# ostadabbas/TePose

Hardware: AMD Instinct MI355X
Metric: 16-frame windows/sec (whole node) (higher is better)
Workload: dtype f32 via 3 fp16 MFMAs on hi+lo halves (22 bits/operand, fp32 acc); exact-f32 MFMA run = value_exact_fp32; 1 GPU; cfg-C synthetic [8192,16,2133] fp32 windows per GPU, TePose n_layers=2 hidden=1024, random-init weights, synthetic SMPL tables, H36M-14 joint path; seqlen=16, parallelism=clip-sharded dp1

## Files before the change

include/tepose_amd.h:

```cpp
#ifndef TEPOSE_AMD_H
#define TEPOSE_AMD_H

#include <stddef.h>
#include <stdint.h>

#ifdef __cplusplus
extern "C" {
#endif

#define TEPOSE_ABI_VERSION 1

#define TEPOSE_E_ARG (-1)
#define TEPOSE_E_SHAPE (-2)
#define TEPOSE_E_WORKSPACE (-3)
#define TEPOSE_E_STATE (-4)
#define TEPOSE_E_TIMEOUT (-5)

#define TEPOSE_FEAT 2048
#define TEPOSE_THETA 85
#define TEPOSE_INPUT 2133
#define TEPOSE_NVERT 6890
#define TEPOSE_NJOINT 24

typedef struct tepose_model tepose_model;
// ... 62 lines not shown
int tepose_project_frame_pair(const tepose_model* m, const float* feat_prev, const float* feat_new, long feat_ld, const float* theta_prev,
                              long theta_ld, int B, float* out_prev, long out_prev_ld, float* out_new, long out_new_ld, void* workspace,
                              size_t ws_bytes, void* stream);
int tepose_window_step(const tepose_model* m, const float* feat_prev, const float* feat_new, long feat_ld, const float* theta_prev, long theta_ld,
                       float* out_prev, long out_prev_ld, float* newest, long newest_ld, const float* ring_base, int ring, int first_slot,
                       long clip_stride, int B, int T, const void* jreg_packed, float* theta, float* verts, float* kp_3d, float* kp_2d, float* rotmat,
                       void* workspace, size_t ws_bytes, void* pair_workspace, size_t pair_ws_bytes, void* stream);
int tepose_forward_cached(const tepose_model* m, const float* ring_base, int ring, int first_slot,
                          long clip_stride, const float* newest, long newest_ld, int B, int T,
                          const void* jreg_packed, float* theta, float* verts, float* kp_3d,
                          float* kp_2d, float* rotmat, void* workspace, size_t ws_bytes, void* stream);

int tepose_create_vibe(int n_layers, int hidden, tepose_model** out);
int tepose_create_vibe_ex(int n_layers, int hidden, int bidirectional, int add_linear, tepose_model** out);
int tepose_pack_vibe_encoder(tepose_model* m, const float* const* w, int n_w, void* stream);
size_t tepose_vibe_workspace_bytes(const tepose_model* m, int B, int N);
int tepose_vibe_feature_dim(const tepose_model* m);
int tepose_vibe_encoder_fwd(const tepose_model* m, const float* x, int B, int N, int use_residual,
                            float* feat, void* workspace, size_t ws_bytes, void* stream);

int tepose_create_hmr(tepose_model** out);
int tepose_pack_hmr_backbone(tepose_model* m, const float* const* w, int n_w, void* stream);
size_t tepose_hmr_workspace_bytes(const tepose_model* m, int N);
int tepose_hmr_features(const tepose_model* m, const float* x, int N, float* feat, void* workspace, size_t ws_bytes, void* stream);

int tepose_metrics_joints(const float* pred, const float* target, int N, int J, int pelvis_mode,
                          float* mpjpe, float* pa_mpjpe, float* accel, void* stream);
int tepose_smpl_verts_from_theta(const tepose_model* m, const float* theta, int N, float* verts,
                                 void* workspace, size_t ws_bytes, void* stream);
int tepose_smpl_fwd(const tepose_model* m, int pose2rot, const float* pose, const float* betas, int N,
                    float* verts, float* joints49, void* workspace, size_t ws_bytes, void* stream);
int tepose_joints_from_verts(const tepose_model* m, const void* jreg_packed, const float* verts, int N, float* kp_3d, void* stream);
int tepose_smpl_fwd_per_person(const tepose_model* m, const float* pose, const float* betas, int N, float* verts,
                               void* workspace, size_t ws_bytes, void* stream);
int tepose_metrics_verts(const float* pred_verts, const float* target_verts, int N, float* mpvpe,
                         void* stream);

int tepose_filter_one_euro(float* x, int N, int D, float min_cutoff, float beta, float d_cutoff,
                           void* stream);
int tepose_filter_slerp(const float* rotmat_in, float* rotmat_out, int N, int J, double ratio,
                        void* stream);

int tepose_rotmat_to_angle_axis(const float* R, int N, float* aa, void* stream);
int tepose_rot6d_to_rotmat(const float* x6, int N, float* R, void* stream);

size_t tepose_gemm_workspace_bytes(int N, int K);
int tepose_gemm_f32(const float* A, long lda, const float* W, long ldw, const float* bias,
                    float* C, long ldc, int M, int N, int K, int relu_a, void* workspace,
                    size_t ws_bytes, void* stream);

size_t tepose_gemm_h3_workspace_bytes(int M, int N, int K);
int tepose_gemm_h3_f32(const float* A, long lda, const float* W, long ldw, const float* bias, float* C,
                       long ldc, int M, int N, int K, void* workspace, size_t ws_bytes, void* stream);

size_t tepose_conv2d_nhwc_workspace_bytes(int N, int H, int W, int Cin, int Cout, int R);
int tepose_conv2d_nhwc_f32(const float* x, int N, int H, int W, int Cin, const float* w_oihw, const float* bias, int Cout, int R,
                           int stride, int pad, int relu_in, const float* residual, float* y, int exact, void* workspace,
                           size_t ws_bytes, void* stream);
int tepose_maxpool3x3s2_nhwc(const float* x, int N, int H, int W, int C, float* y, void* stream);
int tepose_avgpool7_nhwc(const float* x, int N, int C, float* y, void* stream);
int tepose_hmr_fold_pack(const float* w_oihw, const float* gamma, const float* beta, const float* mean, const float* var, int Cout,
                         int Cin, int R, float* w_out, float* b_out, void* stream);

int tepose_profile_enable(tepose_model* m, int on);
int tepose_profile_read(tepose_model* m, double* total_ms, int* n_launches, double* flops_per_launch);
int tepose_profile_read_gru(tepose_model* m, double* total_ms, int* n_forwards, double* flops_per_forward);
int tepose_profile_read_l1proj(tepose_model* m, double* total_ms, int* n_forwards, double* flops_per_forward);

#ifdef __cplusplus
}
#endif
#endif
```

tepose_amd/_lib.py:

```python
import ctypes
import os
from ctypes import c_uint, POINTER, c_char_p, c_double, c_float, c_int, c_int32, c_long, c_size_t, c_void_p

_HERE = os.path.dirname(os.path.abspath(__file__))
LIB_PATH = (os.environ.get("TEPOSE_AMD_LIB") or os.path.join(_HERE, 'libtepose_hip.so'))

SYMBOLS = [
    'tepose_version', 'tepose_error_string', 'tepose_create', 'tepose_destroy',
    'tepose_packed_bytes', 'tepose_set_blob', 'tepose_adopt_blob', 'tepose_pack_encoder', 'tepose_pack_regressor',
    'tepose_pack_smpl', 'tepose_jreg_packed_bytes', 'tepose_pack_jreg', 'tepose_workspace_bytes',
    'tepose_encoder_fwd', 'tepose_regressor_fwd', 'tepose_forward', 'tepose_gemm_workspace_bytes',
    'tepose_gemm_f32', 'tepose_profile_enable', 'tepose_profile_read', 'tepose_create_vibe', 'tepose_create_vibe_ex', 'tepose_vibe_feature_dim',
    'tepose_pack_vibe_encoder', 'tepose_vibe_workspace_bytes', 'tepose_vibe_encoder_fwd',
    'tepose_metrics_joints', 'tepose_smpl_verts_from_theta', 'tepose_metrics_verts', 'tepose_smpl_fwd', 'tepose_filter_one_euro', 'tepose_filter_slerp', 'tepose_project_frames', 'tepose_project_frame_pair', 'tepose_window_step', 'tepose_forward_cached', 'tepose_profile_read_gru', 'tepose_profile_read_l1proj', 'tepose_gemm_h3_workspace_bytes', 'tepose_gemm_h3_f32',
    'tepose_regressor_fwd_init', 'tepose_rotmat_to_angle_axis', 'tepose_rot6d_to_rotmat',
    'tepose_project_frames_workspace_bytes', 'tepose_smpl_fwd_per_person', 'tepose_joints_from_verts',
    'tepose_status', 'tepose_forward_status', 'tepose_status_peek', 'tepose_fault_code', 'tepose_set_persistent', 'tepose_uses_persistent', 'tepose_build_info',
    'tepose_fp32_ranges', 'tepose_derive_planes', 'tepose_kernel_info', 'tepose_select_kernels', 'tepose_set_option', 'tepose_get_option', 'tepose_debug_set_test_fault', 'tepose_debug_kernel_errors',
    'tepose_create_hmr', 'tepose_pack_hmr_backbone', 'tepose_hmr_workspace_bytes', 'tepose_hmr_features', 'tepose_conv2d_nhwc_workspace_bytes',
    'tepose_conv2d_nhwc_f32', 'tepose_maxpool3x3s2_nhwc', 'tepose_avgpool7_nhwc', 'tepose_hmr_fold_pack',
]

_lib = None


class TeposeError(RuntimeError):
    pass


E_TIMEOUT = -5


class TeposeTimeout(TeposeError):
    """TEPOSE_E_TIMEOUT: a persistent small-batch kernel gave up waiting for its peers (GPU shared or CU-masked);
    the outputs of that forward are NaN.  Engine re-runs on the step-per-launch kernels where it owns the sync point."""


class TeposeKernelFault(TeposeError):
    """(A sibling of TeposeTimeout, not a subclass: the retry loops that catch TeposeTimeout -- run_clips, StreamSession -- must not re-run on it.)
    The fault channel reported code 4: a bounded LDS poll of the barrier-free projection kernel (csrc/gemm_h3s16c.hip) expired.  No wait in that
    kernel depends on another workgroup, so this is a kernel bug or a hardware fault -- not a shared / CU-masked GPU, and the persistent small-batch
    kernels have nothing to do with it.  The forward's outputs are invalid (NaN-poisoned); the handle stays as it is."""


def load():
    global _lib
    if _lib is not None:
        return _lib
    if not os.path.isfile(LIB_PATH):
        raise ImportError(
            'tepose_amd: %s not found. Build it with `python -c "import __graft_entry__ as g; '
            'g.build()"` (hipcc --offload-arch=gfx950). There is no fallback path.' % LIB_PATH)
    lib = ctypes.CDLL(LIB_PATH)
    fp = c_void_p
    lib.tepose_version.restype = c_int
    lib.tepose_error_string.restype = c_char_p
    lib.tepose_error_string.argtypes = [c_int]
    lib.tepose_create.argtypes = [c_int, c_int, POINTER(c_void_p)]
    lib.tepose_destroy.argtypes = [c_void_p]
    lib.tepose_destroy.restype = None
    lib.tepose_packed_bytes.argtypes = [c_void_p]
    lib.tepose_packed_bytes.restype = c_size_t
    lib.tepose_set_blob.argtypes = [c_void_p, fp, c_size_t]
    lib.tepose_adopt_blob.argtypes = [c_void_p]
    lib.tepose_pack_encoder.argtypes = [c_void_p, POINTER(c_void_p), c_int, c_void_p]
    lib.tepose_pack_regressor.argtypes = [c_void_p, POINTER(c_void_p), c_int, c_void_p]
    lib.tepose_pack_smpl.argtypes = [c_void_p, fp, fp, fp, fp, fp, fp, POINTER(c_int32), c_void_p]
    lib.tepose_jreg_packed_bytes.restype = c_size_t
    lib.tepose_pack_jreg.argtypes = [fp, fp, c_void_p]
    lib.tepose_workspace_bytes.argtypes = [c_void_p, c_int, c_int]
    lib.tepose_workspace_bytes.restype = c_size_t
    lib.tepose_encoder_fwd.argtypes = [c_void_p, fp, c_int, c_int, c_int, fp, fp, c_size_t, c_void_p]
    lib.tepose_regressor_fwd.argtypes = [c_void_p, fp, c_int, c_int, fp, fp, fp, fp, fp, fp, fp,
                                         c_size_t, c_void_p]
    lib.tepose_forward.argtypes = [c_void_p, fp, c_int, c_int, fp, fp, fp, fp, fp, fp, fp, c_size_t,
                                   c_void_p]
    lib.tepose_regressor_fwd_init.argtypes = [c_void_p, fp, c_int, c_int, fp, fp, fp, fp, fp, fp, fp, fp, fp, fp,
                                              c_size_t, c_void_p]
    lib.tepose_rotmat_to_angle_axis.argtypes = [fp, c_int, fp, c_void_p]
    lib.tepose_rot6d_to_rotmat.argtypes = [fp, c_int, fp, c_void_p]
    lib.tepose_gemm_workspace_bytes.argtypes = [c_int, c_int]
    lib.tepose_gemm_workspace_bytes.restype = c_size_t
    lib.tepose_gemm_f32.argtypes = [fp, c_long, fp, c_long, fp, fp, c_long, c_int, c_int, c_int, c_int,
                                    fp, c_size_t, c_void_p]
    lib.tepose_create_vibe.argtypes = [c_int, c_int, POINTER(c_void_p)]
    lib.tepose_create_vibe_ex.argtypes = [c_int, c_int, c_int, c_int, POINTER(c_void_p)]
    lib.tepose_vibe_feature_dim.argtypes = [c_void_p]
    lib.tepose_pack_vibe_encoder.argtypes = [c_void_p, POINTER(c_void_p), c_int, c_void_p]
    lib.tepose_vibe_workspace_bytes.argtypes = [c_void_p, c_int, c_int]
    lib.tepose_vibe_workspace_bytes.restype = c_size_t
    lib.tepose_vibe_encoder_fwd.argtypes = [c_void_p, fp, c_int, c_int, c_int, fp, fp, c_size_t, c_void_p]
    lib.tepose_metrics_joints.argtypes = [fp, fp, c_int, c_int, c_int, fp, fp, fp, c_void_p]
    lib.tepose_smpl_verts_from_theta.argtypes = [c_void_p, fp, c_int, fp, fp, c_size_t, c_void_p]
    lib.tepose_metrics_verts.argtypes = [fp, fp, c_int, fp, c_void_p]
    lib.tepose_smpl_fwd.argtypes = [c_void_p, c_int, fp, fp, c_int, fp, fp, fp, c_size_t, c_void_p]
    lib.tepose_smpl_fwd_per_person.argtypes = [c_void_p, fp, fp, c_int, fp, fp, c_size_t, c_void_p]
    lib.tepose_filter_one_euro.argtypes = [fp, c_int, c_int, c_float, c_float, c_float, c_void_p]
    lib.tepose_filter_slerp.argtypes = [fp, fp, c_int, c_int, c_double, c_void_p]
    lib.tepose_project_frames_workspace_bytes.argtypes = [c_void_p, c_int]
    lib.tepose_project_frames_workspace_bytes.restype = c_size_t
    lib.tepose_project_frames.argtypes = [c_void_p, fp, c_long, fp, c_long, c_int, fp, c_long, fp, c_size_t, c_void_p]
    lib.tepose_project_frame_pair.argtypes = [c_void_p, fp, fp, c_long, fp, c_long, c_int, fp, c_long, fp, c_long, fp, c_size_t, c_void_p]
    lib.tepose_window_step.argtypes = [c_void_p, fp, fp, c_long, fp, c_long, fp, c_long, fp, c_long, fp, c_int, c_int, c_long, c_int, c_int, fp, fp, fp, fp, fp, fp,
                                       fp, c_size_t, fp, c_size_t, c_void_p]
    lib.tepose_forward_cached.argtypes = [c_void_p, fp, c_int, c_int, c_long, fp, c_long, c_int, c_int, fp, fp, fp, fp,
                                          fp, fp, fp, c_size_t, c_void_p]
    lib.tepose_gemm_h3_workspace_bytes.argtypes = [c_int, c_int, c_int]
    lib.tepose_gemm_h3_workspace_bytes.restype = c_size_t
    lib.tepose_gemm_h3_f32.argtypes = [fp, c_long, fp, c_long, fp, fp, c_long, c_int, c_int, c_int, fp, c_size_t, c_void_p]
    lib.tepose_fp32_ranges.argtypes = [c_void_p, POINTER(c_size_t), POINTER(c_size_t), c_int]
    lib.tepose_derive_planes.argtypes = [c_void_p, c_void_p]
    lib.tepose_status.argtypes = [c_void_p, c_void_p]
    lib.tepose_forward_status.argtypes = [c_void_p, c_void_p, c_void_p]
    lib.tepose_debug_set_test_fault.argtypes = [c_void_p, c_uint]
    lib.tepose_debug_kernel_errors.restype = c_uint
    lib.tepose_status_peek.argtypes = [c_void_p]
    lib.tepose_fault_code.argtypes = [c_void_p]
    lib.tepose_set_persistent.argtypes = [c_void_p, c_int]
    lib.tepose_uses_persistent.argtypes = [c_void_p, c_int, c_int]
    lib.tepose_joints_from_verts.argtypes = [c_void_p, fp, fp, c_int, fp, c_void_p]
    lib.tepose_profile_enable.argtypes = [c_void_p, c_int]
    lib.tepose_profile_read.argtypes = [c_void_p, POINTER(c_double), POINTER(c_int), POINTER(c_double)]
    lib.tepose_profile_read_gru.argtypes = [c_void_p, POINTER(c_double), POINTER(c_int), POINTER(c_double)]
    lib.tepose_profile_read_l1proj.argtypes = [c_void_p, POINTER(c_double), POINTER(c_int), POINTER(c_double)]
    lib.tepose_create_hmr.argtypes = [POINTER(c_void_p)]
    lib.tepose_pack_hmr_backbone.argtypes = [c_void_p, POINTER(c_void_p), c_int, c_void_p]
    lib.tepose_hmr_workspace_bytes.argtypes = [c_void_p, c_int]
    lib.tepose_hmr_workspace_bytes.restype = c_size_t
    lib.tepose_hmr_features.argtypes = [c_void_p, fp, c_int, fp, fp, c_size_t, c_void_p]
    lib.tepose_conv2d_nhwc_workspace_bytes.argtypes = [c_int] * 6
    lib.tepose_conv2d_nhwc_workspace_bytes.restype = c_size_t
    lib.tepose_conv2d_nhwc_f32.argtypes = [fp, c_int, c_int, c_int, c_int, fp, fp, c_int, c_int, c_int, c_int, c_int, fp, fp, c_int, fp, c_size_t, c_void_p]
    lib.tepose_maxpool3x3s2_nhwc.argtypes = [fp, c_int, c_int, c_int, c_int, fp, c_void_p]
    lib.tepose_avgpool7_nhwc.argtypes = [fp, c_int, c_int, fp, c_void_p]
    lib.tepose_hmr_fold_pack.argtypes = [fp, fp, fp, fp, fp, c_int, c_int, c_int, fp, fp, c_void_p]
    for name in SYMBOLS:
        getattr(lib, name)
    if lib.tepose_version() != 1:
        raise ImportError('tepose_amd: ABI version mismatch (%d)' % lib.tepose_version())
    lib.tepose_build_info.restype = c_char_p
    lib.tepose_kernel_info.restype = c_char_p
    lib.tepose_kernel_info.argtypes = [c_void_p]
    lib.tepose_select_kernels.restype = c_char_p
    lib.tepose_set_option.argtypes = [c_void_p, c_char_p, ctypes.c_long]
    lib.tepose_get_option.argtypes = [c_void_p, c_char_p]
    lib.tepose_get_option.restype = ctypes.c_long
    lib.tepose_select_kernels.argtypes = [c_void_p, c_int, c_int]
    info = (lib.tepose_build_info() or b'').decode()
    if 'packed_fp32=off' not in info:
        import warnings
        warnings.warn('tepose_amd: %s was built WITH packed-fp32 VALU instructions (%r); on a GPU shared by two processes such a '
                      'build returned wrong SMPL vertices in 1-3 %% of the launches (DESIGN.md section 10) -- rebuild with '
                      '__graft_entry__.build()' % (LIB_PATH, info), RuntimeWarning)
    _lib = lib
    return lib


def check(rc, what):
    if rc != 0:
        msg = load().tepose_error_string(rc)
        raise (TeposeTimeout if rc == E_TIMEOUT else TeposeError)('%s failed: %s (code %d)' % (what, msg.decode() if msg else '?', rc))

# ... 5 lines not shown
```

tepose_amd/csrc/api.hip:

```cpp
#include <stdlib.h>
#include <string.h>

#include <new>

#include "plan.h"

using namespace tepose;

static inline void fault_collected(const tepose_model* m) {
  std::lock_guard<std::mutex> g(m->q_mu);
  ++m->collected;
}

static void read_env_knobs(tepose_model* m) {
  m->opt = options_from_env();
  const char* e = getenv("TEPOSE_EXACT_FP32");
  m->split = m->split_env = !(e && atoi(e) != 0);
  e = getenv("TEPOSE_LARGE_BATCH_KERNELS");
  m->large_scaled = !(e && std::string(e) == "twoacc");
  e = getenv("TEPOSE_GRU_STATE");
  m->state_planes = !(e && std::string(e) == "fp32");
  e = getenv("TEPOSE_COLLAPSE_REGRESSOR");
  m->collapse_env = !(e && atoi(e) == 0);
  e = getenv("TEPOSE_S_MIN_B");
// ... 267 lines not shown
}

int tepose_metrics_verts(const float* pred_verts, const float* target_verts, int N, float* mpvpe, void* stream) {
  if (!pred_verts || !target_verts || !mpvpe || N < 1) return TEPOSE_E_ARG;
  CK(launch_metrics_verts(pred_verts, target_verts, N, mpvpe, (hipStream_t)stream));
  return 0;
}

int tepose_filter_one_euro(float* x, int N, int D, float min_cutoff, float beta, float d_cutoff, void* stream) {
  if (!x || N < 1 || D < 1) return TEPOSE_E_ARG;
  CK(launch_one_euro(x, N, D, min_cutoff, beta, d_cutoff, (hipStream_t)stream));
  return 0;
}

int tepose_filter_slerp(const float* rotmat_in, float* rotmat_out, int N, int J, double ratio, void* stream) {
  if (!rotmat_in || !rotmat_out || N < 1 || J < 1) return TEPOSE_E_ARG;
  CK(launch_slerp_smooth(rotmat_in, rotmat_out, N, J, ratio, (hipStream_t)stream));
  return 0;
}

int tepose_rotmat_to_angle_axis(const float* R, int N, float* aa, void* stream) {
  if (!R || !aa || N < 1) return TEPOSE_E_ARG;
  CK(launch_rotmat_to_aa(R, N, aa, (hipStream_t)stream));
  return 0;
}

int tepose_rot6d_to_rotmat(const float* x6, int N, float* R, void* stream) {
  if (!x6 || !R || N < 1) return TEPOSE_E_ARG;
  CK(launch_rot6d_to_rotmat(x6, N, R, (hipStream_t)stream));
  return 0;
}

size_t tepose_gemm_h3_workspace_bytes(int M, int N, int K) {
  if (M < 1 || N < 1 || K < 1) return 0;
  const size_t a = gemm_h3_ws_bytes(M, N, K), b = gemm_h3s_ws_bytes(M, N, K);
  return a > b ? a : b;
}

int tepose_gemm_h3_f32(const float* A, long lda, const float* W, long ldw, const float* bias, float* C, long ldc,
                       int M, int N, int K, void* workspace, size_t ws_bytes, void* stream) {
  if (!A || !W || !C || !workspace || M < 1 || N < 1 || K < 1) return TEPOSE_E_ARG;
  if (K % 32 != 0) return TEPOSE_E_SHAPE;
  if (ws_bytes < gemm_h3_ws_bytes(M, N, K)) return TEPOSE_E_WORKSPACE;
  const char* pe = getenv("TEPOSE_H3S");
  const Options opt = options_from_env();
  if (pe && pe[0] && std::string(pe) != "0" && std::string(pe).rfind("skinny", 0) != 0 && ws_bytes >= gemm_h3s_ws_bytes(M, N, K)) {
    CK(launch_gemm_h3s_f32(A, lda, W, ldw, C, ldc, M, N, K, 256.f, 16384.f, workspace, (hipStream_t)stream, opt, bias, std::string(pe) == "mid" ? 1 : 0));
    return 0;
  }
  CK(launch_gemm_h3_f32(A, lda, W, ldw, bias, C, ldc, M, N, K, workspace, (hipStream_t)stream, opt, pe && std::string(pe) == "skinny" ? 1 : 0));
  return 0;
}

size_t tepose_gemm_workspace_bytes(int N, int K) {
  if (N < 1 || K < 1) return 0;
  return (size_t)round_up(N, 128) * round_up(K, 32) * sizeof(float) + 256;
}

int tepose_gemm_f32(const float* A, long lda, const float* W, long ldw, const float* bias, float* C, long ldc,
                    int M, int N, int K, int relu_a, void* workspace, size_t ws_bytes, void* stream) {
  if (!A || !W || !C || !workspace || M < 1 || N < 1 || K < 1) return TEPOSE_E_ARG;
  if (lda % 4 != 0 || ((uintptr_t)A & 15) != 0 || K % 32 != 0) return TEPOSE_E_SHAPE;
  if (ws_bytes < tepose_gemm_workspace_bytes(N, K)) return TEPOSE_E_WORKSPACE;
  hipStream_t s = (hipStream_t)stream;
  float* wp = (float*)workspace;
  CK((hipError_t)pack(W, ldw, N, K, wp, round_up(N, 128), K, 0, 0, 0, 1, s));
  const GemmArgs g{A, lda, wp, K, C, ldc, bias, nullptr, 0, 1.f, M, N, relu_a};
  CK(launch_gemm(g, s, options_from_env()));
  return 0;
}

}
```

tepose_amd/csrc/common.h:

```cpp
#pragma once
#include <hip/hip_runtime.h>
#include <stdint.h>

namespace tepose {

typedef _Float16 half_t;
constexpr float kLoScale = 2048.f;
__host__ __device__ inline void split_hi_lo(float a, half_t& hi, half_t& lo) {
  hi = (half_t)a;
  lo = (half_t)((a - (float)hi) * kLoScale);
}

constexpr int kFeat = 2048;
constexpr int kTheta = 85;
constexpr int kInput = 2133;
constexpr int kInputP = 2144;
constexpr int kNV = 6890;
constexpr int kNJ = 24;
constexpr int kNPose = 144;
constexpr int kState = 160;
constexpr int kBlendK = 224;
constexpr int kBlendN = 20736;
constexpr int kVertLd = 20672;

// ... 228 lines not shown
  int N, n_iter;
};
hipError_t launch_reg_seq(const RegSeqArgs& a, hipStream_t s);
bool gru_seq_ok(int ndir, int M, int Hp, int T, const Options& o);
int gru_seq_gran_rows(const Options& o);
hipError_t launch_gru_seq(const GruSeqArgs& a, hipStream_t s, const Options& o);
struct GateBatch { GateDir d[3]; };
hipError_t launch_gru_first(const GateBatch& gb, int ndir, int M, int Hp, hipStream_t s, int scaled16 = 0, bool rows16 = false);
hipError_t launch_split_planes(const float* src, long ld, long rows, int K, int Kp, long R, void* hi, void* lo,
                               hipStream_t s, int relu = 0);
struct RowPairSrc { const float* f0; const float* th0; const float* f1; long fld, thld; long B; };
hipError_t launch_split_rows(const float* src, long ld, long rows, int K, int Kp, long R, int fmt16, void* hi, void* lo,
                             float* row_scale, hipStream_t s, bool few, void* zero = nullptr, size_t zero_bytes = 0,
                             int permT = 0, const RowPairSrc* pair = nullptr);
hipError_t launch_gemm_h3_f32(const float* A, long lda, const float* W, long ldw, const float* bias, float* C,
                              long ldc, int M, int N, int K, void* ws, hipStream_t s, const Options& o, int kind = 0);
size_t gemm_h3_ws_bytes(int M, int N, int K);
__host__ __device__ inline long plane16_index(long row, long k, long R) {
  return ((k >> 4) * R + row) * 16 + ((((k >> 3) & 1) ^ ((row >> 3) & 1)) << 3) + (k & 7);
}
constexpr float kStateScale = 16384.f;
struct H3SArgs {
  const half_t *Ah, *Al; long a_kst;
  const half_t *Wh, *Wl; long w_kst;
  int Kp;
  float* C; long ldc;
  const float* bias;
  float inv_scale;
  int M, N;
  const float* row_scale;
  unsigned* status = nullptr;
  unsigned* fault = nullptr;
  unsigned inject = 0;
  int c_blk_hp = 0;
};
struct H3SBatch { H3SArgs p[3]; GateDir gate[3]; int n; int Hp; float state_scale; };
hipError_t launch_gemm_h3s(const H3SArgs& a, hipStream_t s, const Options& o, int tag = 1);
bool gemm_h3s16_ok(const H3SArgs& a);
hipError_t launch_gemm_h3s16c(const H3SArgs& a, hipStream_t s, int tag, int gm);
unsigned h3s16c_read_err();
void h3s16c_warm();
bool gru_step16_ok(const H3SBatch& b);
bool gru_step16_planes_ok(const H3SBatch& b);
hipError_t launch_gru_step16(const H3SBatch& b, hipStream_t s, bool planes, int gm);
unsigned* h3s16c_err_of_device();
bool gemm_h3s_mid_ok(const H3SArgs& a);
hipError_t launch_gemm_h3s_mid(const H3SArgs& a, hipStream_t s);
hipError_t launch_split_planes16(const float* src, long ld, long rows, int K, int Kp, long R, float p, void* hi,
                                 void* lo, hipStream_t s);
hipError_t launch_absmax(const float* src, size_t n, float* out, hipStream_t s);
size_t gemm_h3s_ws_bytes(int M, int N, int K);
hipError_t launch_gemm_h3s_f32(const float* A, long lda, const float* W, long ldw, float* C, long ldc, int M, int N,
                               int K, float pA, float pW, void* ws, hipStream_t s, const Options& o, const float* bias = nullptr,
                               int mid = 0);

}
```

tepose_amd/csrc/gemm_h3s.hip:

```cpp
#include <type_traits>

#include "common.h"


namespace tepose {

typedef float f32x16 __attribute__((ext_vector_type(16)));
typedef _Float16 h16x8 __attribute__((ext_vector_type(8)));

__device__ __forceinline__ void glds16s(const void* g, void* l) {
  __builtin_amdgcn_global_load_lds((const __attribute__((address_space(1))) void*)g,
                                   (__attribute__((address_space(3))) void*)l, 16, 0, 0);
}
template <int N>
__device__ __forceinline__ void wait_vms() {
  asm volatile("s_waitcnt vmcnt(%0)" ::"n"(N) : "memory");
}

__global__ void __launch_bounds__(256) split_planes16_kernel(const float* __restrict__ src, long ld, long rows, int K,
                                                             int Kp, long R, float p, _Float16* __restrict__ hi,
                                                             _Float16* __restrict__ lo) {
  typedef _Float16 h16x2s __attribute__((ext_vector_type(2)));
  const int KT = Kp / 16;
  const long units = ((rows + 7) / 8) * KT;
// ... 192 lines not shown
    for (int i = 0; i < WMF; ++i)
#pragma unroll
      for (int j = 0; j < WNT; ++j) acc[i][j] = __builtin_amdgcn_mfma_f32_32x32x16_f16(al[i], bh[j], acc[i][j], 0, 0, 0);
  };
  int kt = 0;
  for (; kt + NST - 1 < KT; ++kt) ktile(kt, std::true_type{});
  for (; kt < KT; ++kt) ktile(kt, std::false_type{});
  wait_vms<0>();

  {
    float bv[WNT];
#pragma unroll
    for (int j = 0; j < WNT; ++j) {
      const int col = n0 + wn * 32 * WNT + j * 32 + r;
      bv[j] = (a.bias && col < a.N) ? a.bias[col] : 0.f;
    }
#pragma unroll
    for (int i = 0; i < WMF; ++i)
#pragma unroll
      for (int e = 0; e < 16; ++e) {
        const int row = m0 + wm * 32 * WMF + i * 32 + (e & 3) + 8 * (e >> 2) + 4 * h;
        if (row >= a.M) continue;
        const float rs = a.row_scale ? a.row_scale[row] * a.inv_scale : a.inv_scale;
#pragma unroll
        for (int j = 0; j < WNT; ++j) {
          const int col = n0 + wn * 32 * WNT + j * 32 + r;
          if (col < a.N) a.C[(long)row * a.ldc + col] = acc[i][j][e] * rs + bv[j];
        }
      }
  }
}

hipError_t launch_gemm_h3s(const H3SArgs& a, hipStream_t s, const Options& o, int tag) {
  if (a.M <= 0 || a.N <= 0) return hipSuccess;
  return launch_gemm_h3s16c(a, s, tag, o.s16_gm);
}

bool gemm_h3s_mid_ok(const H3SArgs& a) { return a.N % 288 == 0 && a.Kp % 16 == 0 && a.M > 0; }
hipError_t launch_gemm_h3s_mid(const H3SArgs& a, hipStream_t s) {
  if (!gemm_h3s_mid_ok(a)) return hipErrorInvalidValue;
  const int tilesM = (a.M + 127) / 128, tilesN = a.N / 288;
  H3SBatch b{};
  b.p[0] = a; b.n = 1;
  hipLaunchKernelGGL((gemm_h3s_kernel<1, 3, 4, 3>), dim3(tilesM * tilesN, 1), dim3(768), 0, s, b, tilesM, tilesN);
  return hipGetLastError();
}

size_t gemm_h3s_ws_bytes(int M, int N, int K) {
  const size_t Kp = (size_t)round_up(K, 16);
  return 2 * align_up((size_t)M * Kp * 2, 256) + 2 * align_up((size_t)round_up(N, 256) * Kp * 2, 256) + 256;
}

hipError_t launch_gemm_h3s_f32(const float* A, long lda, const float* W, long ldw, float* C, long ldc, int M, int N,
                               int K, float pA, float pW, void* ws, hipStream_t s, const Options& o, const float* bias, int mid) {
  const int Kp = round_up(K, 16), Np = round_up(N, 256);
  char* p = (char*)ws;
  _Float16* Ah = (_Float16*)p; p += align_up((size_t)M * Kp * 2, 256);
  _Float16* Al = (_Float16*)p; p += align_up((size_t)M * Kp * 2, 256);
  _Float16* Wh = (_Float16*)p; p += align_up((size_t)Np * Kp * 2, 256);
  _Float16* Wl = (_Float16*)p;
  hipError_t e = hipMemsetAsync(Wh, 0, 2 * align_up((size_t)Np * Kp * 2, 256), s);
  if (e != hipSuccess) return e;
  if ((e = launch_split_planes16(A, lda, M, K, Kp, M, pA, Ah, Al, s)) != hipSuccess) return e;
  if ((e = launch_split_planes16(W, ldw, N, K, Kp, Np, pW, Wh, Wl, s)) != hipSuccess) return e;
  H3SArgs a{Ah, Al, (long)M * 16, Wh, Wl, (long)Np * 16, Kp, C, ldc, bias, 1.f / (pA * pW), M, N};
  if (mid) return launch_gemm_h3s_mid(a, s);
  return launch_gemm_h3s(a, s, o);
}

}
```

tepose_amd/csrc/gemm_h3s16c.hip:

```cpp
#include "common.h"

#ifndef TEPOSE_C_VAR
#define TEPOSE_C_VAR 5
#endif

namespace tepose {

typedef float f32x4c __attribute__((ext_vector_type(4)));
typedef _Float16 h16x8c __attribute__((ext_vector_type(8)));

__device__ __forceinline__ void h3s16c_tile_of_block(int bid, int nwg, int tilesM, int tilesN, int& tm, int& tn, int GM) {
  const int q = nwg >> 3, r = nwg & 7, xcd = bid & 7, loc = bid >> 3;
  const int lin = (xcd < r ? xcd * (q + 1) : r * (q + 1) + (xcd - r) * q) + loc;
  const int group = lin / (GM * tilesN), rem = lin - group * GM * tilesN;
  const int gm = min(GM, tilesM - group * GM);
  tm = group * GM + rem % gm;
  tn = rem / gm;
}

template <int TAG>
__global__ void __launch_bounds__(512) gemm_h3s_persist16c_kernel(H3SArgs a, int tilesM, int tilesN, int GM, unsigned* err) {
  constexpr int NWN = 2, NST = 4, MT = 4, NT = 8;
  constexpr int HM = 256, HN = 256, HK = 16, RB = HK * 2, RPI = 1024 / RB;
  constexpr int STAGE = (2 * HM + 2 * HN) * RB, TOT = STAGE / 1024, Q = TOT / 8;
  constexpr int SPIN = 1 << 18;
  __shared__ __attribute__((aligned(16))) char lds[NST * STAGE + 64];
  const int ntiles = tilesM * tilesN;
  const int tid = threadIdx.x, lane = tid & 63, wave = __builtin_amdgcn_readfirstlane(tid >> 6);
  const int wm = wave / NWN, wn = wave % NWN;
  const int t = lane & 15, g = lane >> 4;
  const unsigned lds0 = (unsigned)(size_t)lds;
  const unsigned cnt0 = lds0 + NST * STAGE;
  if (tid < 16) ((unsigned*)(lds + NST * STAGE))[tid] = 0u;
  __syncthreads();
  auto fresh_lane = [&]() __attribute__((always_inline)) {
    int l = lane;
    asm volatile("" : "+v"(l));
    return l;
  };
  const int i0 = wave * Q;
  bool isA[Q];
  int lrow0[Q];
  long kst[Q];
  const char* pbase[Q];
#pragma unroll
  for (int q = 0; q < Q; ++q) {
    int ri = (i0 + q) * RPI;
    isA[q] = ri < 2 * HM;
    if (!isA[q]) ri -= 2 * HM;
    const bool lo = ri >= (isA[q] ? HM : HN);
    lrow0[q] = lo ? ri - (isA[q] ? HM : HN) : ri;
    pbase[q] = (const char*)(isA[q] ? (lo ? a.Al : a.Ah) : (lo ? a.Wl : a.Wh));
    kst[q] = (isA[q] ? a.a_kst : a.w_kst) * 2;
  }
  const char* sbase[Q];
  unsigned voff[Q];
  int m0 = 0, n0 = 0;
  auto setup = [&](int tile) {
    int tm, tn;
    h3s16c_tile_of_block(tile, ntiles, tilesM, tilesN, tm, tn, GM);
    m0 = tm * HM; n0 = tn * HN;
    const int l = fresh_lane();
#pragma unroll
    for (int q = 0; q < Q; ++q) {
      const int grow = isA[q] ? min(m0 + lrow0[q] + l / 2, a.M - 1) : n0 + lrow0[q] + l / 2;
      voff[q] = (unsigned)grow * RB + 16u * (l & 1);
      sbase[q] = pbase[q];
    }
  };
  auto request_pair = [&](int pair) __attribute__((always_inline)) {
#pragma unroll
    for (int s = 0; s < 2; ++s)
#pragma unroll
      for (int q = 0; q < Q; ++q) {
        const unsigned dst = lds0 + (unsigned)((((2 * pair + s) % NST) * STAGE) + (i0 + q) * 1024);
        asm volatile("s_mov_b32 m0, %2\n\ts_nop 0\n\tglobal_load_lds_dwordx4 %0, %1" : : "v"(voff[q]), "s"(sbase[q]), "s"(dst) : "m0", "memory");
        sbase[q] += kst[q];
      }
  };
  auto bump = [&](int slot) __attribute__((always_inline)) {
    if (lane == 0) asm volatile("ds_add_u32 %0, %1" : : "v"(cnt0 + 4u * (unsigned)slot), "v"(1u) : "memory");
  };
  bool dead = false;
  const unsigned INJ = a.inject;
  auto poll = [&](int slot, int target) __attribute__((always_inline)) {
    const unsigned addr = cnt0 + 4u * (unsigned)slot;
    for (int spins = 0;; ++spins) {
      unsigned v;
      asm volatile("ds_read_b32 %0, %1\n\ts_waitcnt lgkmcnt(0)" : "=v"(v) : "v"(addr) : "memory");
      if ((int)((unsigned)__builtin_amdgcn_readfirstlane((int)v) - (unsigned)target - INJ) >= 0) break;
      if (spins > SPIN) { dead = true; break; }
      __builtin_amdgcn_s_sleep(1);
    }
  };
  const unsigned sx = 16u * ((g & 1) ^ ((t >> 3) & 1)) + (unsigned)(g >> 1) * STAGE;
  const unsigned abase = lds0 + (unsigned)(wm * 16 * MT + t) * RB + sx;
  const unsigned bbase = lds0 + 2 * HM * RB + (unsigned)(wn * 16 * NT + t) * RB + sx;
  constexpr int A_LO = HM * RB, W_LO = HN * RB;
  const int NP = a.Kp / (2 * HK);
  const bool vec = (((size_t)a.C | (size_t)a.bias) & 15) == 0 && (a.ldc & 3) == 0;

  f32x4c acc[MT][NT];
  h16x8c ah[MT], al[MT], bh[2][2], bl[2][2];
#define TEPOSE_C_READ_A(AB)                                                                                                   \
  _Pragma("unroll") for (int i = 0; i < MT; ++i) {                                                                            \
    asm volatile("ds_read_b128 %0, %1 offset:%2" : "=v"(ah[i]) : "v"(AB), "n"(i * 16 * RB));                                  \
    asm volatile("ds_read_b128 %0, %1 offset:%2" : "=v"(al[i]) : "v"(AB), "n"(i * 16 * RB + A_LO));                           \
  }
#define TEPOSE_C_READ_B(BB, QD)                                                                                               \
  _Pragma("unroll") for (int u = 0; u < 2; ++u) {                                                                             \
    asm volatile("ds_read_b128 %0, %1 offset:%2" : "=v"(bh[(QD) & 1][u]) : "v"(BB), "n"((2 * (QD) + u) * 16 * RB));          \
    asm volatile("ds_read_b128 %0, %1 offset:%2" : "=v"(bl[(QD) & 1][u]) : "v"(BB), "n"((2 * (QD) + u) * 16 * RB + W_LO));   \
  }
#define TEPOSE_C_WAIT_B(N, X)                                                                                                 \
  asm volatile("s_waitcnt lgkmcnt(" #N ")" : "+v"(bh[X][0]), "+v"(bh[X][1]), "+v"(bl[X][0]), "+v"(bl[X][1]) : : "memory")
  auto request_one = [&](int pair, int k) __attribute__((always_inline)) {
    const int sgi = k / Q, q = k % Q;
    const unsigned dst = lds0 + (unsigned)((((2 * pair + sgi) % NST) * STAGE) + (i0 + q) * 1024);
    asm volatile("s_mov_b32 m0, %2\n\ts_nop 0\n\tglobal_load_lds_dwordx4 %0, %1" : : "v"(voff[q]), "s"(sbase[q]), "s"(dst) : "m0", "memory");
    sbase[q] += kst[q];
  };
  auto quarter = [&](int QD, int X, bool dma = false, int pair = 0) __attribute__((always_inline)) {
#pragma unroll
    for (int i = 0; i < MT; ++i)
#pragma unroll
      for (int u = 0; u < 2; ++u) {
        acc[i][2 * QD + u] = __builtin_amdgcn_mfma_f32_16x16x32_f16(bh[X][u], ah[i], acc[i][2 * QD + u], 0, 0, 0);
        if (dma) request_one(pair, i * 2 + u);
      }
#pragma unroll
    for (int i = 0; i < MT; ++i)
#pragma unroll
      for (int u = 0; u < 2; ++u) acc[i][2 * QD + u] = __builtin_amdgcn_mfma_f32_16x16x32_f16(bl[X][u], ah[i], acc[i][2 * QD + u], 0, 0, 0);
#pragma unroll
    for (int i = 0; i < MT; ++i)
#pragma unroll
      for (int u = 0; u < 2; ++u) acc[i][2 * QD + u] = __builtin_amdgcn_mfma_f32_16x16x32_f16(bh[X][u], al[i], acc[i][2 * QD + u], 0, 0, 0);
  };

  int tile = blockIdx.x;
  if (tile >= ntiles) return;
  setup(tile);
  int dtile = tile, dpt = 0;
  request_pair(0);
  ++dpt;
  asm volatile("s_waitcnt vmcnt(0)" ::: "memory");
  bump(0);
#pragma unroll
  for (int i = 0; i < MT; ++i)
#pragma unroll
    for (int j = 0; j < NT; ++j) acc[i][j] = f32x4c{0.f, 0.f, 0.f, 0.f};
  int pt = 0, gp = 0;
  int tm0 = m0, tn0 = n0;
  for (;;) {
    poll(gp & 1, 8 * (gp / 2 + 1));
    if (dead) break;
    bool requested = false;
    if (dpt >= NP) {
      const int nt = dtile + (int)gridDim.x;
      if (nt < ntiles) { dtile = nt; dpt = 0; setup(nt); }
    }
    if (dpt < NP) {
      if (!(TEPOSE_C_VAR & 4)) request_pair(gp + 1);
      ++dpt; requested = true;
    }
    const unsigned par = (unsigned)(gp & 1) * 2u * STAGE;
    const unsigned ab = abase + par, bb = bbase + par;
    TEPOSE_C_READ_A(ab)
    TEPOSE_C_READ_B(bb, 0)
    TEPOSE_C_READ_B(bb, 1)
    asm volatile("s_waitcnt lgkmcnt(4)"
                 : "+v"(ah[0]), "+v"(ah[1]), "+v"(ah[2]), "+v"(ah[3]), "+v"(al[0]), "+v"(al[1]), "+v"(al[2]), "+v"(al[3]),
                   "+v"(bh[0][0]), "+v"(bh[0][1]), "+v"(bl[0][0]), "+v"(bl[0][1])
                 :
                 : "memory");
    __builtin_amdgcn_sched_barrier(0);
    if ((TEPOSE_C_VAR & 4) && requested) quarter(0, 0, true, gp + 1); else quarter(0, 0);
    __builtin_amdgcn_sched_barrier(0);
    TEPOSE_C_READ_B(bb, 2)
    TEPOSE_C_WAIT_B(4, 1);
    __builtin_amdgcn_sched_barrier(0);
    quarter(1, 1);
    __builtin_amdgcn_sched_barrier(0);
    TEPOSE_C_READ_B(bb, 3)
    TEPOSE_C_WAIT_B(4, 0);
    auto confirm = [&]() __attribute__((always_inline)) {
      if (requested) {
        asm volatile("s_waitcnt vmcnt(0)" ::: "memory");
        bump((gp + 1) & 1);
      }
    };
    if ((TEPOSE_C_VAR & 3) == 1) confirm();
    __builtin_amdgcn_sched_barrier(0);
    quarter(2, 0);
    __builtin_amdgcn_sched_barrier(0);
    TEPOSE_C_WAIT_B(0, 1);
    if ((TEPOSE_C_VAR & 3) == 0) confirm();
    __builtin_amdgcn_sched_barrier(0);
    quarter(3, 1);
    __builtin_amdgcn_sched_barrier(0);
    if ((TEPOSE_C_VAR & 3) == 2) confirm();
    ++gp;
    if (pt + 1 < NP) { ++pt; continue; }

    const int le = fresh_lane(), te = le & 15, ge = le >> 4;
    const bool full = tm0 + HM <= a.M && tn0 + HN <= a.N && vec;
    if (full) {
      float rs[MT];
#pragma unroll
      for (int i = 0; i < MT; ++i) {
        const int row = tm0 + wm * 16 * MT + i * 16 + te;
        rs[i] = a.row_scale ? a.row_scale[row] * a.inv_scale : a.inv_scale;
      }
      float* c0 = a.C + (long)(tm0 + wm * 16 * MT + te) * a.ldc + tn0 + wn * 16 * NT + 4 * ge;
      const float* b0 = a.bias ? a.bias + tn0 + wn * 16 * NT + 4 * ge : nullptr;
      if (a.c_blk_hp) {
        const long rt_stride = (long)a.N * 16;
        float* cb = a.C + (long)((tm0 + wm * 16 * MT) >> 4) * rt_stride + le * 4;
        const int col0 = tn0 + wn * 16 * NT;
#pragma unroll
        for (int j = 0; j < NT; ++j) {
          const f32x4c bq = b0 ? *(const f32x4c*)(b0 + j * 16) : f32x4c{0.f, 0.f, 0.f, 0.f};
          float* cj = cb + gi_blk_col_block(col0 + j * 16, a.c_blk_hp);
#pragma unroll
          for (int i = 0; i < MT; ++i) {
            f32x4c v;
#pragma unroll
            for (int c = 0; c < 4; ++c) v[c] = acc[i][j][c] * rs[i] + bq[c];
            *(f32x4c*)(cj + (long)i * rt_stride) = v;
          }
        }
      } else {
#pragma unroll
      for (int j = 0; j < NT; ++j) {
        const f32x4c bq = b0 ? *(const f32x4c*)(b0 + j * 16) : f32x4c{0.f, 0.f, 0.f, 0.f};
#pragma unroll
        for (int i = 0; i < MT; ++i) {
          f32x4c v;
#pragma unroll
          for (int c = 0; c < 4; ++c) v[c] = acc[i][j][c] * rs[i] + bq[c];
          *(f32x4c*)(c0 + (long)i * 16 * a.ldc + j * 16) = v;
        }
      }
      }
    } else {
#pragma unroll
      for (int i = 0; i < MT; ++i) {
        const int row = tm0 + wm * 16 * MT + i * 16 + te;
        if (row >= a.M) continue;
        const float rsv = a.row_scale ? a.row_scale[row] * a.inv_scale : a.inv_scale;
#pragma unroll
        for (int j = 0; j < NT; ++j)
#pragma unroll
          for (int c = 0; c < 4; ++c) {
            const int col = tn0 + wn * 16 * NT + j * 16 + 4 * ge + c;
            if (col < a.N) {
              const float v = acc[i][j][c] * rsv + (a.bias ? a.bias[col] : 0.f);
              if (a.c_blk_hp) a.C[(long)(row >> 4) * a.N * 16 + gi_blk_col_block(col & ~15, a.c_blk_hp) + ((((col & 15) >> 2) * 16 + (row & 15)) << 2) + (col & 3)] = v;
              else a.C[(long)row * a.ldc + col] = v;
            }
          }
      }
    }
    const int next = tile + (int)gridDim.x;
    if (next >= ntiles) break;
    tile = next;
    tm0 = m0; tn0 = n0;
    pt = 0;
#pragma unroll
    for (int i = 0; i < MT; ++i)
#pragma unroll
      for (int j = 0; j < NT; ++j) acc[i][j] = f32x4c{0.f, 0.f, 0.f, 0.f};
  }
#undef TEPOSE_C_READ_A
#undef TEPOSE_C_READ_B
#undef TEPOSE_C_WAIT_B
  if (dead && lane == 0) {
    if (err) atomicAdd(err, 1u);
    a.C[0] = __builtin_nanf("");
    if (a.status) __hip_atomic_store(a.status, 4u, __ATOMIC_RELAXED, __HIP_MEMORY_SCOPE_AGENT);
    if (a.fault) __hip_atomic_store(a.fault, 4u, __ATOMIC_RELAXED, __HIP_MEMORY_SCOPE_SYSTEM);
  }
}

static constexpr int kMaxDev = 64;
static unsigned* g_h3s16c_err[kMaxDev] = {};

unsigned* h3s16c_err_of_device() {
  int dev = -1;
  if (hipGetDevice(&dev) != hipSuccess || dev < 0 || dev >= kMaxDev) { (void)hipGetLastError(); return nullptr; }
  return __atomic_load_n(&g_h3s16c_err[dev], __ATOMIC_ACQUIRE);
}

void h3s16c_warm() {
  int dev = -1;
  if (hipGetDevice(&dev) != hipSuccess || dev < 0 || dev >= kMaxDev) { (void)hipGetLastError(); return; }
  if (__atomic_load_n(&g_h3s16c_err[dev], __ATOMIC_ACQUIRE)) return;
  unsigned* q = nullptr;
  if (hipMalloc((void**)&q, 256) != hipSuccess || !q) { (void)hipGetLastError(); return; }
  (void)hipMemset(q, 0, 256);
  unsigned* expected = nullptr;
  if (!__atomic_compare_exchange_n(&g_h3s16c_err[dev], &expected, q, false, __ATOMIC_RELEASE, __ATOMIC_ACQUIRE)) (void)hipFree(q);
}

bool gemm_h3s16_ok(const H3SArgs& a) { return a.Kp % 32 == 0 && a.Kp >= 64; }

hipError_t launch_gemm_h3s16c(const H3SArgs& a, hipStream_t s, int tag, int gm_opt) {
  if (a.M <= 0 || a.N <= 0) return hipSuccess;
  if (!gemm_h3s16_ok(a)) return hipErrorInvalidValue;
  const int tilesM = (a.M + 255) / 256, tilesN = (a.N + 255) / 256;
  const int nt = tilesM * tilesN;
  const int gm = gm_opt >= 1 && gm_opt <= 32 ? gm_opt : 8;
  unsigned* err = h3s16c_err_of_device();
  if (tag == 0) hipLaunchKernelGGL(gemm_h3s_persist16c_kernel<0>, dim3(nt < 256 ? nt : 256), dim3(512), 0, s, a, tilesM, tilesN, gm, err);
  else hipLaunchKernelGGL(gemm_h3s_persist16c_kernel<1>, dim3(nt < 256 ? nt : 256), dim3(512), 0, s, a, tilesM, tilesN, gm, err);
  return hipGetLastError();
}

unsigned h3s16c_read_err() {
  unsigned total = 0;
  for (int d = 0; d < kMaxDev; ++d) {
    unsigned* p = __atomic_load_n(&g_h3s16c_err[d], __ATOMIC_ACQUIRE);
    unsigned v = 0;
    if (p && hipMemcpy(&v, p, 4, hipMemcpyDeviceToHost) == hipSuccess) total += v;
  }
// ... 5 lines not shown
```

Baseline: 294,000 windows/s.

## Overlap GEMM tile epilogue stores with next tile's MFMA loop in persistent kernel

Bit 8 is now set in the default variant. With it, the persistent h3s16c GEMM stores only the first column slice of a tile at the tile boundary, after staging row scales and bias in LDS. The remaining output slices are stored between MFMAs during the first three quarters of the next tile's first K step, and the confirm wait relaxes to vmcnt(8) while stores are pending. The change also collapses the per-unit DMA address arrays into one base offset with clamping, swaps per-iteration LDS parity arithmetic for an incremental flip, and exposes a public row-scaled, blocked-output h3s entry point. In exchange it uses more LDS and registers and adds more interleaved memory traffic inside the main loop.

```diff
diff --git a/include/tepose_amd.h b/include/tepose_amd.h
--- a/include/tepose_amd.h
+++ b/include/tepose_amd.h
@@ -138,6 +138,8 @@
 size_t tepose_gemm_h3_workspace_bytes(int M, int N, int K);
 int tepose_gemm_h3_f32(const float* A, long lda, const float* W, long ldw, const float* bias, float* C,
                        long ldc, int M, int N, int K, void* workspace, size_t ws_bytes, void* stream);
+int tepose_gemm_h3s_f32(const float* A, long lda, const float* W, long ldw, const float* bias, const float* row_scale, float* C,
+                        long ldc, int M, int N, int K, int c_blk_hp, void* workspace, size_t ws_bytes, void* stream);
 
 size_t tepose_conv2d_nhwc_workspace_bytes(int N, int H, int W, int Cin, int Cout, int R);
 int tepose_conv2d_nhwc_f32(const float* x, int N, int H, int W, int Cin, const float* w_oihw, const float* bias, int Cout, int R,
diff --git a/tepose_amd/_lib.py b/tepose_amd/_lib.py
--- a/tepose_amd/_lib.py
+++ b/tepose_amd/_lib.py
@@ -12,7 +12,7 @@
     'tepose_encoder_fwd', 'tepose_regressor_fwd', 'tepose_forward', 'tepose_gemm_workspace_bytes',
     'tepose_gemm_f32', 'tepose_profile_enable', 'tepose_profile_read', 'tepose_create_vibe', 'tepose_create_vibe_ex', 'tepose_vibe_feature_dim',
     'tepose_pack_vibe_encoder', 'tepose_vibe_workspace_bytes', 'tepose_vibe_encoder_fwd',
-    'tepose_metrics_joints', 'tepose_smpl_verts_from_theta', 'tepose_metrics_verts', 'tepose_smpl_fwd', 'tepose_filter_one_euro', 'tepose_filter_slerp', 'tepose_project_frames', 'tepose_project_frame_pair', 'tepose_window_step', 'tepose_forward_cached', 'tepose_profile_read_gru', 'tepose_profile_read_l1proj', 'tepose_gemm_h3_workspace_bytes', 'tepose_gemm_h3_f32',
+    'tepose_metrics_joints', 'tepose_smpl_verts_from_theta', 'tepose_metrics_verts', 'tepose_smpl_fwd', 'tepose_filter_one_euro', 'tepose_filter_slerp', 'tepose_project_frames', 'tepose_project_frame_pair', 'tepose_window_step', 'tepose_forward_cached', 'tepose_profile_read_gru', 'tepose_profile_read_l1proj', 'tepose_gemm_h3_workspace_bytes', 'tepose_gemm_h3_f32', 'tepose_gemm_h3s_f32',
     'tepose_regressor_fwd_init', 'tepose_rotmat_to_angle_axis', 'tepose_rot6d_to_rotmat',
     'tepose_project_frames_workspace_bytes', 'tepose_smpl_fwd_per_person', 'tepose_joints_from_verts',
     'tepose_status', 'tepose_forward_status', 'tepose_status_peek', 'tepose_fault_code', 'tepose_set_persistent', 'tepose_uses_persistent', 'tepose_build_info',
@@ -108,6 +108,7 @@
     lib.tepose_gemm_h3_workspace_bytes.argtypes = [c_int, c_int, c_int]
     lib.tepose_gemm_h3_workspace_bytes.restype = c_size_t
     lib.tepose_gemm_h3_f32.argtypes = [fp, c_long, fp, c_long, fp, fp, c_long, c_int, c_int, c_int, fp, c_size_t, c_void_p]
+    lib.tepose_gemm_h3s_f32.argtypes = [fp, c_long, fp, c_long, fp, fp, fp, c_long, c_int, c_int, c_int, c_int, fp, c_size_t, c_void_p]
     lib.tepose_fp32_ranges.argtypes = [c_void_p, POINTER(c_size_t), POINTER(c_size_t), c_int]
     lib.tepose_derive_planes.argtypes = [c_void_p, c_void_p]
     lib.tepose_status.argtypes = [c_void_p, c_void_p]
diff --git a/tepose_amd/csrc/api.hip b/tepose_amd/csrc/api.hip
--- a/tepose_amd/csrc/api.hip
+++ b/tepose_amd/csrc/api.hip
@@ -343,6 +343,16 @@
   return 0;
 }
 
+int tepose_gemm_h3s_f32(const float* A, long lda, const float* W, long ldw, const float* bias, const float* row_scale, float* C, long ldc,
+                        int M, int N, int K, int c_blk_hp, void* workspace, size_t ws_bytes, void* stream) {
+  if (!A || !W || !C || !workspace || M < 1 || N < 1 || K < 1 || c_blk_hp < 0) return TEPOSE_E_ARG;
+  if (K % 32 != 0 || K < 64) return TEPOSE_E_SHAPE;
+  if (c_blk_hp && (c_blk_hp % 16 != 0 || N % (3 * c_blk_hp) != 0 || M % 16 != 0 || ldc != N)) return TEPOSE_E_SHAPE;
+  if (ws_bytes < gemm_h3s_ws_bytes(M, N, K)) return TEPOSE_E_WORKSPACE;
+  CK(launch_gemm_h3s_f32(A, lda, W, ldw, C, ldc, M, N, K, 256.f, 16384.f, workspace, (hipStream_t)stream, options_from_env(), bias, 0, row_scale, c_blk_hp));
+  return 0;
+}
+
 size_t tepose_gemm_workspace_bytes(int N, int K) {
   if (N < 1 || K < 1) return 0;
   return (size_t)round_up(N, 128) * round_up(K, 32) * sizeof(float) + 256;
diff --git a/tepose_amd/csrc/common.h b/tepose_amd/csrc/common.h
--- a/tepose_amd/csrc/common.h
+++ b/tepose_amd/csrc/common.h
@@ -304,6 +304,7 @@
 size_t gemm_h3s_ws_bytes(int M, int N, int K);
 hipError_t launch_gemm_h3s_f32(const float* A, long lda, const float* W, long ldw, float* C, long ldc, int M, int N,
                                int K, float pA, float pW, void* ws, hipStream_t s, const Options& o, const float* bias = nullptr,
-                               int mid = 0);
-
-}
+                               int mid = 0,
+                               const float* row_scale = nullptr, int c_blk_hp = 0);
+
+}
diff --git a/tepose_amd/csrc/gemm_h3s.hip b/tepose_amd/csrc/gemm_h3s.hip
--- a/tepose_amd/csrc/gemm_h3s.hip
+++ b/tepose_amd/csrc/gemm_h3s.hip
@@ -268,7 +268,8 @@
 }
 
 hipError_t launch_gemm_h3s_f32(const float* A, long lda, const float* W, long ldw, float* C, long ldc, int M, int N,
-                               int K, float pA, float pW, void* ws, hipStream_t s, const Options& o, const float* bias, int mid) {
+                               int K, float pA, float pW, void* ws, hipStream_t s, const Options& o, const float* bias, int mid,
+                               const float* row_scale, int c_blk_hp) {
   const int Kp = round_up(K, 16), Np = round_up(N, 256);
   char* p = (char*)ws;
   _Float16* Ah = (_Float16*)p; p += align_up((size_t)M * Kp * 2, 256);
@@ -281,6 +282,8 @@
   if ((e = launch_split_planes16(W, ldw, N, K, Kp, Np, pW, Wh, Wl, s)) != hipSuccess) return e;
   H3SArgs a{Ah, Al, (long)M * 16, Wh, Wl, (long)Np * 16, Kp, C, ldc, bias, 1.f / (pA * pW), M, N};
   if (mid) return launch_gemm_h3s_mid(a, s);
+  a.row_scale = row_scale;
+  a.c_blk_hp = c_blk_hp;
   return launch_gemm_h3s(a, s, o);
 }
 
diff --git a/tepose_amd/csrc/gemm_h3s16c.hip b/tepose_amd/csrc/gemm_h3s16c.hip
--- a/tepose_amd/csrc/gemm_h3s16c.hip
+++ b/tepose_amd/csrc/gemm_h3s16c.hip
@@ -1,7 +1,7 @@
 #include "common.h"
 
 #ifndef TEPOSE_C_VAR
-#define TEPOSE_C_VAR 5
+#define TEPOSE_C_VAR 13
 #endif
 
 namespace tepose {
@@ -24,7 +24,8 @@
   constexpr int HM = 256, HN = 256, HK = 16, RB = HK * 2, RPI = 1024 / RB;
   constexpr int STAGE = (2 * HM + 2 * HN) * RB, TOT = STAGE / 1024, Q = TOT / 8;
   constexpr int SPIN = 1 << 18;
-  __shared__ __attribute__((aligned(16))) char lds[NST * STAGE + 64];
+  constexpr int EPF = 64 + 16 * NT;
+  __shared__ __attribute__((aligned(16))) char lds[NST * STAGE + 64 + 8 * EPF * 4];
   const int ntiles = tilesM * tilesN;
   const int tid = threadIdx.x, lane = tid & 63, wave = __builtin_amdgcn_readfirstlane(tid >> 6);
   const int wm = wave / NWN, wn = wave % NWN;
@@ -39,34 +40,25 @@
     return l;
   };
   const int i0 = wave * Q;
-  bool isA[Q];
-  int lrow0[Q];
-  long kst[Q];
-  const char* pbase[Q];
-#pragma unroll
-  for (int q = 0; q < Q; ++q) {
-    int ri = (i0 + q) * RPI;
-    isA[q] = ri < 2 * HM;
-    if (!isA[q]) ri -= 2 * HM;
-    const bool lo = ri >= (isA[q] ? HM : HN);
-    lrow0[q] = lo ? ri - (isA[q] ? HM : HN) : ri;
-    pbase[q] = (const char*)(isA[q] ? (lo ? a.Al : a.Ah) : (lo ? a.Wl : a.Wh));
-    kst[q] = (isA[q] ? a.a_kst : a.w_kst) * 2;
-  }
-  const char* sbase[Q];
-  unsigned voff[Q];
+  static_assert(HM == HN && (HM * RB / 1024) % Q == 0, "a wave's units must not straddle two planes");
+  int ri0 = i0 * RPI;
+  const bool isA = ri0 < 2 * HM;
+  if (!isA) ri0 -= 2 * HM;
+  const bool lo = ri0 >= HM;
+  const int lrow0 = lo ? ri0 - HM : ri0;
+  const char* const pbase = (const char*)(isA ? (lo ? a.Al : a.Ah) : (lo ? a.Wl : a.Wh));
+  const long kst = (isA ? a.a_kst : a.w_kst) * 2;
+  const char* sbase = pbase;
+  unsigned voff0 = 0, vmax = 0;
   int m0 = 0, n0 = 0;
   auto setup = [&](int tile) {
     int tm, tn;
     h3s16c_tile_of_block(tile, ntiles, tilesM, tilesN, tm, tn, GM);
     m0 = tm * HM; n0 = tn * HN;
     const int l = fresh_lane();
-#pragma unroll
-    for (int q = 0; q < Q; ++q) {
-      const int grow = isA[q] ? min(m0 + lrow0[q] + l / 2, a.M - 1) : n0 + lrow0[q] + l / 2;
-      voff[q] = (unsigned)grow * RB + 16u * (l & 1);
-      sbase[q] = pbase[q];
-    }
+    vmax = isA ? (unsigned)(a.M - 1) * RB + 16u * (l & 1) : ~0u;
+    voff0 = min((unsigned)((isA ? m0 : n0) + lrow0 + l / 2) * RB + 16u * (l & 1), vmax);
+    sbase = pbase;
   };
   auto request_pair = [&](int pair) __attribute__((always_inline)) {
 #pragma unroll
@@ -74,8 +66,8 @@
 #pragma unroll
       for (int q = 0; q < Q; ++q) {
         const unsigned dst = lds0 + (unsigned)((((2 * pair + s) % NST) * STAGE) + (i0 + q) * 1024);
-        asm volatile("s_mov_b32 m0, %2\n\ts_nop 0\n\tglobal_load_lds_dwordx4 %0, %1" : : "v"(voff[q]), "s"(sbase[q]), "s"(dst) : "m0", "memory");
-        sbase[q] += kst[q];
+        asm volatile("s_mov_b32 m0, %2\n\ts_nop 0\n\tglobal_load_lds_dwordx4 %0, %1" : : "v"(min(voff0 + 1024u * q, vmax)), "s"(sbase), "s"(dst) : "m0", "memory");
+        if (q == Q - 1) sbase += kst;
       }
   };
   auto bump = [&](int slot) __attribute__((always_inline)) {
@@ -94,8 +86,8 @@
     }
   };
   const unsigned sx = 16u * ((g & 1) ^ ((t >> 3) & 1)) + (unsigned)(g >> 1) * STAGE;
-  const unsigned abase = lds0 + (unsigned)(wm * 16 * MT + t) * RB + sx;
-  const unsigned bbase = lds0 + 2 * HM * RB + (unsigned)(wn * 16 * NT + t) * RB + sx;
+  unsigned ab = lds0 + (unsigned)(wm * 16 * MT + t) * RB + sx;
+  unsigned bb = lds0 + 2 * HM * RB + (unsigned)(wn * 16 * NT + t) * RB + sx;
   constexpr int A_LO = HM * RB, W_LO = HN * RB;
   const int NP = a.Kp / (2 * HK);
   const bool vec = (((size_t)a.C | (size_t)a.bias) & 15) == 0 && (a.ldc & 3) == 0;
@@ -114,18 +106,49 @@
   }
 #define TEPOSE_C_WAIT_B(N, X)                                                                                                 \
   asm volatile("s_waitcnt lgkmcnt(" #N ")" : "+v"(bh[X][0]), "+v"(bh[X][1]), "+v"(bl[X][0]), "+v"(bl[X][1]) : : "memory")
+  float* const ep = (float*)(lds + NST * STAGE + 64) + wave * EPF;
+  char* ecb = nullptr;
+  auto epi_stage = [&](int tm, int tn) __attribute__((always_inline)) {
+    const int l = fresh_lane();
+    ep[l] = a.row_scale ? a.row_scale[tm + wm * 16 * MT + l] * a.inv_scale : a.inv_scale;
+    float b0v = 0.f, b1v = 0.f;
+    if (a.bias) { const float* bp = a.bias + tn + wn * 16 * NT + 2 * l; b0v = bp[0]; b1v = bp[1]; }
+    ep[64 + 2 * l] = b0v;
+    ep[64 + 2 * l + 1] = b1v;
+    const int on0 = tn + wn * 16 * NT;
+    ecb = (char*)(a.c_blk_hp ? a.C + (long)((tm + wm * 16 * MT) >> 4) * ((long)a.N * 16) + gi_blk_col_block(on0, a.c_blk_hp)
+                             : a.C + (long)(tm + wm * 16 * MT) * a.ldc + on0);
+    asm volatile("" ::: "memory");
+    __builtin_amdgcn_wave_barrier();
+  };
+  auto epi_one = [&](int QD, int k) __attribute__((always_inline)) {
+    const int i = k % MT, u = k / MT, j = 2 * QD + u;
+    const int l = fresh_lane();
+    const bool blk = a.c_blk_hp != 0;
+    const unsigned eoff = blk ? (unsigned)l * 16u : ((unsigned)(l & 15) * (unsigned)a.ldc + 4u * (unsigned)(l >> 4)) * 4u;
+    const long istride = blk ? (long)a.N * 16 : 16 * a.ldc;
+    char* ub = ecb + ((long)i * istride + (blk ? (long)gi_blk_block(0, j * 16) : (long)j * 16)) * 4;
+    const float rs = ep[i * 16 + (l & 15)];
+    const f32x4c bq = *(const f32x4c*)(ep + 64 + j * 16 + 4 * (l >> 4));
+#pragma unroll
+    for (int c = 0; c < 4; ++c) acc[i][j][c] = acc[i][j][c] * rs + bq[c];
+    *(f32x4c*)(ub + eoff) = acc[i][j];
+    acc[i][j] = f32x4c{0.f, 0.f, 0.f, 0.f};
+    asm volatile("" ::: "memory");
+  };
   auto request_one = [&](int pair, int k) __attribute__((always_inline)) {
     const int sgi = k / Q, q = k % Q;
     const unsigned dst = lds0 + (unsigned)((((2 * pair + sgi) % NST) * STAGE) + (i0 + q) * 1024);
-    asm volatile("s_mov_b32 m0, %2\n\ts_nop 0\n\tglobal_load_lds_dwordx4 %0, %1" : : "v"(voff[q]), "s"(sbase[q]), "s"(dst) : "m0", "memory");
-    sbase[q] += kst[q];
-  };
-  auto quarter = [&](int QD, int X, bool dma = false, int pair = 0) __attribute__((always_inline)) {
+    asm volatile("s_mov_b32 m0, %2\n\ts_nop 0\n\tglobal_load_lds_dwordx4 %0, %1" : : "v"(min(voff0 + 1024u * q, vmax)), "s"(sbase), "s"(dst) : "m0", "memory");
+    if (q == Q - 1) sbase += kst;
+  };
+  auto quarter = [&](int QD, int X, bool dma = false, int pair = 0, bool pend = false, int epi = -1) __attribute__((always_inline)) {
 #pragma unroll
     for (int i = 0; i < MT; ++i)
 #pragma unroll
       for (int u = 0; u < 2; ++u) {
         acc[i][2 * QD + u] = __builtin_amdgcn_mfma_f32_16x16x32_f16(bh[X][u], ah[i], acc[i][2 * QD + u], 0, 0, 0);
+        if (epi >= 0 && __builtin_expect(pend, 0)) epi_one(epi, i * 2 + u);
         if (dma) request_one(pair, i * 2 + u);
       }
 #pragma unroll
@@ -164,8 +187,7 @@
       if (!(TEPOSE_C_VAR & 4)) request_pair(gp + 1);
       ++dpt; requested = true;
     }
-    const unsigned par = (unsigned)(gp & 1) * 2u * STAGE;
-    const unsigned ab = abase + par, bb = bbase + par;
+    const bool pend = ecb != nullptr;
     TEPOSE_C_READ_A(ab)
     TEPOSE_C_READ_B(bb, 0)
     TEPOSE_C_READ_B(bb, 1)
@@ -175,24 +197,26 @@
                  :
                  : "memory");
     __builtin_amdgcn_sched_barrier(0);
-    if ((TEPOSE_C_VAR & 4) && requested) quarter(0, 0, true, gp + 1); else quarter(0, 0);
+    if ((TEPOSE_C_VAR & 4) && requested) quarter(0, 0, true, gp + 1, pend, 1); else quarter(0, 0);
     __builtin_amdgcn_sched_barrier(0);
     TEPOSE_C_READ_B(bb, 2)
     TEPOSE_C_WAIT_B(4, 1);
     __builtin_amdgcn_sched_barrier(0);
-    quarter(1, 1);
+    quarter(1, 1, false, 0, pend, 2);
     __builtin_amdgcn_sched_barrier(0);
     TEPOSE_C_READ_B(bb, 3)
     TEPOSE_C_WAIT_B(4, 0);
     auto confirm = [&]() __attribute__((always_inline)) {
       if (requested) {
-        asm volatile("s_waitcnt vmcnt(0)" ::: "memory");
+        if (pend && (TEPOSE_C_VAR & 7) == 5) asm volatile("s_waitcnt vmcnt(8)" ::: "memory");
+        else asm volatile("s_waitcnt vmcnt(0)" ::: "memory");
         bump((gp + 1) & 1);
       }
     };
     if ((TEPOSE_C_VAR & 3) == 1) confirm();
     __builtin_amdgcn_sched_barrier(0);
-    quarter(2, 0);
+    quarter(2, 0, false, 0, pend, 3);
+    ecb = nullptr;
     __builtin_amdgcn_sched_barrier(0);
     TEPOSE_C_WAIT_B(0, 1);
     if ((TEPOSE_C_VAR & 3) == 0) confirm();
@@ -200,12 +224,21 @@
     quarter(3, 1);
     __builtin_amdgcn_sched_barrier(0);
     if ((TEPOSE_C_VAR & 3) == 2) confirm();
+    {
+      const unsigned flip = (gp & 1) ? 0u - 2u * STAGE : 2u * STAGE;
+      ab += flip; bb += flip;
+    }
     ++gp;
     if (pt + 1 < NP) { ++pt; continue; }
 
     const int le = fresh_lane(), te = le & 15, ge = le >> 4;
     const bool full = tm0 + HM <= a.M && tn0 + HN <= a.N && vec;
-    if (full) {
+    const int next = tile + (int)gridDim.x;
+    if ((TEPOSE_C_VAR & 8) && full && next < ntiles && a.c_blk_hp % (16 * NT) == 0 && a.ldc < (1L << 26)) {
+      epi_stage(tm0, tn0);
+#pragma unroll
+      for (int k = 0; k < 2 * MT; ++k) epi_one(0, k);
+    } else if (full) {
       float rs[MT];
 #pragma unroll
       for (int i = 0; i < MT; ++i) {
@@ -262,15 +295,16 @@
           }
       }
     }
-    const int next = tile + (int)gridDim.x;
     if (next >= ntiles) break;
     tile = next;
     tm0 = m0; tn0 = n0;
     pt = 0;
-#pragma unroll
-    for (int i = 0; i < MT; ++i)
-#pragma unroll
-      for (int j = 0; j < NT; ++j) acc[i][j] = f32x4c{0.f, 0.f, 0.f, 0.f};
+    if (!ecb) {
+#pragma unroll
+      for (int i = 0; i < MT; ++i)
+#pragma unroll
+        for (int j = 0; j < NT; ++j) acc[i][j] = f32x4c{0.f, 0.f, 0.f, 0.f};
+    }
   }
 #undef TEPOSE_C_READ_A
 #undef TEPOSE_C_READ_B
```

Measured after the change: 285,900 windows/s. 2.7% lower.
